# neuraloperator/neuraloperator

Hardware: AMD Instinct MI355X
Metric: FNO SpectralConv fwd+bwd samples/sec (higher is better)
Workload: dtype f32; 1 GPU; fno2d_256_m64_c64_b32; B_per_gpu=32, global_batch=32, channels=64, parallelism=single, launch=eager, real_tensor_io=f32, weights=dense complex64, random init

## Files before the change

include/sc_engine.h:

```cpp
#ifndef SC_ENGINE_H
#define SC_ENGINE_H

#include <stddef.h>
#include <stdint.h>

#ifdef __cplusplus
extern "C" {
#endif

#define SC_MAX_DIMS 4

enum { SC_NORM_FORWARD = 0, SC_NORM_BACKWARD = 1, SC_NORM_ORTHO = 2 };

enum {
  SC_FWD_SCALED = 0,
  SC_FWD_ADJ_C2R = 1,
  SC_INV_PADDED = 0,
  SC_INV_ADJ_R2C = 1
};

typedef struct sc_plan sc_plan;

typedef struct {
  int32_t ndim;
// ... 20 lines not shown
};

int sc_plan_create(sc_plan** out, const sc_plan_desc* desc);
void sc_plan_destroy(sc_plan* plan);
size_t sc_plan_workspace_bytes(const sc_plan* plan, int64_t n_images);
int sc_plan_is_fast(const sc_plan* plan);

int sc_transform_forward(const sc_plan* plan, int mode, const float* x, float* xhat,
                         int64_t n_images, void* workspace, void* stream);

int sc_transform_inverse(const sc_plan* plan, int mode, const float* yhat, const float* bias,
                         int64_t channels, float* y, int64_t n_images, void* workspace,
                         void* stream);

enum {
  SC_GEMM_FORCE_VALU = 1,
  SC_GEMM_STREAM_C = 2,
  SC_GEMM_PAIRED = 4,
  SC_GEMM_WIDE = 8,
  SC_GEMM_NO_STREAM = 16,
  SC_GEMM_NO_SB = 64,
  SC_GEMM_SB_WM4 = 128,
  SC_GEMM_SB_ALT_ORDER = 1 << 25,
  SC_GEMM_NO_FMX = 1 << 24,
  SC_GEMM_F16 = 32
};
#define SC_GEMM_GRID(n) (((n) & 0xffff) << 8)

typedef struct {
  int64_t P, Q, R, n_modes;
  int64_t a_sp, a_sr, a_sm;
  int64_t b_sr, b_sq, b_sm;
  int64_t c_sp, c_sq, c_sm;
  int32_t conj_a, conj_b;
  int32_t accumulate;
  int32_t flags;
  const int32_t* b_idx;
  const int32_t* c_idx;
  int64_t a_sg, b_sg, c_sg;
} sc_modegemm_desc;

int sc_modegemm(const sc_modegemm_desc* d, const float* A, const float* B, float* C,
                void* stream);
int sc_modegemm_pair(const sc_modegemm_desc* d0, const float* A0, const float* B0, float* C0,
                     const sc_modegemm_desc* d1, const float* A1, const float* B1, float* C1, void* stream);
int sc_modegemm_pair_fused(const sc_modegemm_desc* d0, const sc_modegemm_desc* d1);
int sc_modegemm_pair_path(const sc_modegemm_desc* d0, const sc_modegemm_desc* d1);
int sc_modegemm_msum(const sc_modegemm_desc* d, const float* A, const float* B, float* C,
                     void* stream);
size_t sc_modegemm_msum_workspace_bytes(const sc_modegemm_desc* d);
int sc_modegemm_msum_ws(const sc_modegemm_desc* d, const float* A, const float* B, float* C, void* workspace,
                        size_t workspace_bytes, void* stream);
int sc_modegemm_msum_path(const sc_modegemm_desc* d);
int sc_modegemm_uses_matrix_cores(const sc_modegemm_desc* d);
int sc_modegemm_path(const sc_modegemm_desc* d);

int sc_round_f16(const float* in, float* out, int64_t n, void* stream);

int sc_wire_pack_c32(const float* spec, void* wire, int64_t n, int64_t c, int64_t k1, int64_t rest, int64_t P,
                     int64_t rows, int64_t w0, void* stream);

int sc_wire_unpack_c32(const void* wire, float* spec, int64_t n, int64_t c, int64_t k1, int64_t rest, int64_t P,
                       int64_t rows, int64_t w0, void* stream);

int sc_bicubic_rows_forward(const float* x, float* y, int64_t images, int64_t rows_in, int64_t w_in, int64_t src_row0,
                            int64_t h_in, int64_t h_out, int64_t w_out, int64_t out_row0, int64_t rows_out, void* stream);
int sc_bicubic_rows_backward(const float* gy, float* gx, int64_t images, int64_t rows_in, int64_t w_in, int64_t src_row0,
                             int64_t h_in, int64_t h_out, int64_t w_out, int64_t out_row0, int64_t rows_out, void* stream);
// ... 187 lines not shown
```

neuraloperator_amd/_lib.py:

```python
import atexit
import ctypes
import os
import sys
from ctypes import (POINTER, Structure, byref, c_char_p, c_int, c_int32, c_int64, c_size_t,
                    c_void_p)

SC_MAX_DIMS = 4
SC_NORM = {"forward": 0, "backward": 1, "ortho": 2}
SC_FWD_SCALED, SC_FWD_ADJ_C2R = 0, 1
SC_INV_PADDED, SC_INV_ADJ_R2C = 0, 1
SC_PLAN_FORCE_GENERIC = 1
SC_PLAN_FFT_GEN2 = 2
SC_PLAN_NO_MDFT = 4
SC_PLAN_COMPLEX = 8
SC_PLAN_IO_BF16 = 16
SC_PLAN_NO_F2P_SMALL = 32
SC_PLAN_F2P_SMALL_ALWAYS = 64
SC_PLAN_NO_SPAN = 128
SC_PLAN_NO_MX_FFT = 256
SC_PLAN_MX_FFT_3TERM = 512
SC_FREQ_DROPPED = -(1 << 63)
SC_GEMM_FORCE_VALU = 1
SC_GEMM_STREAM_C = 2
SC_GEMM_PAIRED = 4
SC_GEMM_WIDE = 8
SC_GEMM_NO_STREAM = 16
SC_GEMM_F16 = 32
SC_GEMM_NO_SB = 64
SC_GEMM_SB_WM4 = 128
SC_GEMM_NO_FMX = 1 << 24
SC_GEMM_SB_ALT_ORDER = 1 << 25


def SC_GEMM_GRID(n):
    return (int(n) & 0xffff) << 8

_HERE = os.path.dirname(os.path.abspath(__file__))
DEFAULT_LIB = os.path.join(_HERE, "libsc_engine.so")


class PlanDesc(Structure):
    _fields_ = [("ndim", c_int32), ("fft_norm", c_int32),
                ("spatial", c_int64 * SC_MAX_DIMS), ("kept", c_int64 * SC_MAX_DIMS),
                ("flags", c_int32), ("real_col", c_int32),
                ("freq", POINTER(c_int64) * SC_MAX_DIMS)]


class AdamwDesc(Structure):
    _fields_ = [("lr", ctypes.c_double), ("beta1", ctypes.c_double), ("beta2", ctypes.c_double),
                ("eps", ctypes.c_double), ("weight_decay", ctypes.c_double), ("step", c_int64),
                ("correct_bias", c_int32), ("reserved", c_int32)]


class SpectrumShards(Structure):
# ... 84 lines not shown
        ptr, self._as_parameter_ = self._as_parameter_, None
        try:
            if ptr is not None and self._lib is not None and not _SHUTDOWN and not _finalizing():
                self._lib.sc_plan_destroy(ptr)
        except Exception:
            pass

    def __del__(self):
        self.destroy()


class ScEngineLib:

    SYMBOLS = ["sc_plan_create", "sc_plan_destroy", "sc_plan_workspace_bytes", "sc_plan_is_fast",
               "sc_transform_forward", "sc_transform_inverse", "sc_modegemm",
               "sc_modegemm_msum", "sc_modegemm_msum_ws", "sc_modegemm_msum_workspace_bytes", "sc_modegemm_msum_path", "sc_modegemm_uses_matrix_cores", "sc_modegemm_path", "sc_bias_grad", "sc_adamw_step",
               "sc_layer_workspace_bytes", "sc_layer_forward", "sc_layer_backward",
               "sc_last_error", "sc_version", "sc_plan_kernel_name", "sc_transform_inverse_ex",
               "sc_layer_forward_ex", "sc_round_f16", "sc_pointwise_mlp_forward", "sc_pointwise_block_forward",
               "sc_pointwise_mlp_backward", "sc_pointwise_mlp_workspace_bytes", "sc_pointwise_linear_forward",
               "sc_pointwise_linear_backward", "sc_pointwise_linear_workspace_bytes", "sc_layer_backward_ex",
               "sc_pointwise_mlp_backward_ex", "sc_tucker_modes_supported", "sc_tucker_modes_forward",
               "sc_tucker_modes_backward", "sc_tucker_modes_workspace_bytes", "sc_modegemm_pair",
               "sc_modegemm_pair_fused", "sc_modegemm_pair_path", "sc_plan_workspace_bytes_sharded", "sc_transform_forward_sharded",
               "sc_transform_inverse_sharded", "sc_bias_grad_sharded", "sc_tucker_chain_forward",
               "sc_tucker_chain_backward", "sc_tucker_chain_workspace_bytes", "sc_tucker_chain_fused_supported",
               "sc_tucker_chain_t3m_bytes", "sc_tucker_chain_forward_fused", "sc_tucker_chain_backward_fused",
               "sc_tucker_chain_backward_fused_workspace_bytes", "sc_peer_window_alloc", "sc_peer_window_open",
               "sc_peer_window_close", "sc_peer_window_free", "sc_peer_all_to_all", "sc_peer_window_control", "sc_pointwise_linear_forward_ex",
               "sc_pointwise_linear_workspace_bytes_ex", "sc_pointwise_linear_backward_ex", "sc_pointwise_block_backward",
               "sc_pointwise_block_backward_supported", "sc_bicubic_rows_forward", "sc_bicubic_rows_backward",
               "sc_wire_pack_c32", "sc_wire_unpack_c32", "sc_legendre_analysis", "sc_legendre_synthesis", "sc_spectral_op"]

    def __init__(self, path=DEFAULT_LIB):
        if not os.path.isfile(path):
            raise EngineError(
                f"{path} not found: the HIP engine is not built. Run "
                "`python -c 'import __graft_entry__ as g; g.build()'` (needs hipcc). "
                "There is no fallback path.")
        self.path = path
        self.lib = ctypes.CDLL(path)
        L = self.lib
        for s in self.SYMBOLS:
            if not hasattr(L, s):
                raise EngineError(f"{path} does not export {s}")
        L.sc_plan_create.argtypes = [POINTER(c_void_p), POINTER(PlanDesc)]
        L.sc_plan_create.restype = c_int
        L.sc_plan_destroy.argtypes = [c_void_p]
        L.sc_plan_destroy.restype = None
        L.sc_plan_workspace_bytes.argtypes = [c_void_p, c_int64]
        L.sc_plan_workspace_bytes.restype = c_size_t
        L.sc_plan_is_fast.argtypes = [c_void_p]
        L.sc_plan_is_fast.restype = c_int
        L.sc_transform_forward.argtypes = [c_void_p, c_int, c_void_p, c_void_p, c_int64,
                                           c_void_p, c_void_p]
        L.sc_transform_forward.restype = c_int
        L.sc_transform_inverse.argtypes = [c_void_p, c_int, c_void_p, c_void_p, c_int64,
                                           c_void_p, c_int64, c_void_p, c_void_p]
        L.sc_transform_inverse.restype = c_int
        L.sc_modegemm.argtypes = [POINTER(ModeGemmDesc), c_void_p, c_void_p, c_void_p, c_void_p]
        L.sc_modegemm.restype = c_int
        L.sc_modegemm_pair.argtypes = [POINTER(ModeGemmDesc), c_void_p, c_void_p, c_void_p,
                                       POINTER(ModeGemmDesc), c_void_p, c_void_p, c_void_p, c_void_p]
        L.sc_modegemm_pair.restype = c_int
        L.sc_modegemm_pair_fused.argtypes = [POINTER(ModeGemmDesc), POINTER(ModeGemmDesc)]
        L.sc_modegemm_pair_fused.restype = c_int
        L.sc_modegemm_pair_path.argtypes = [POINTER(ModeGemmDesc), POINTER(ModeGemmDesc)]
        L.sc_modegemm_pair_path.restype = c_int
        L.sc_modegemm_msum.argtypes = [POINTER(ModeGemmDesc), c_void_p, c_void_p, c_void_p, c_void_p]
        L.sc_modegemm_msum.restype = c_int
        L.sc_modegemm_msum_workspace_bytes.argtypes = [POINTER(ModeGemmDesc)]
        L.sc_modegemm_msum_workspace_bytes.restype = c_size_t
        L.sc_modegemm_msum_ws.argtypes = [POINTER(ModeGemmDesc), c_void_p, c_void_p, c_void_p, c_void_p, c_size_t, c_void_p]
        L.sc_modegemm_msum_ws.restype = c_int
        L.sc_modegemm_msum_path.argtypes = [POINTER(ModeGemmDesc)]
        L.sc_modegemm_msum_path.restype = c_int
        L.sc_modegemm_uses_matrix_cores.argtypes = [POINTER(ModeGemmDesc)]
        L.sc_modegemm_uses_matrix_cores.restype = c_int
        L.sc_modegemm_path.argtypes = [POINTER(ModeGemmDesc)]
        L.sc_modegemm_path.restype = c_int
        L.sc_bias_grad.argtypes = [c_void_p, c_void_p, c_int64, c_int64, c_void_p, c_void_p]
        L.sc_bias_grad.restype = c_int
        L.sc_plan_workspace_bytes_sharded.argtypes = [c_void_p, c_int64]
        L.sc_plan_workspace_bytes_sharded.restype = c_size_t
        L.sc_transform_forward_sharded.argtypes = [c_void_p, c_int, c_void_p, c_void_p, c_int64,
                                                   POINTER(SpectrumShards), c_void_p, c_void_p]
        L.sc_transform_forward_sharded.restype = c_int
# ... 174 lines not shown

    def modegemm(self, a_ptr, b_ptr, c_ptr, stream=0, **kw):
        self._check(self.lib.sc_modegemm(byref(self._gemm_desc(kw)), a_ptr, b_ptr, c_ptr, stream))

    _DESC_CACHE = {}

    @staticmethod
    def _gemm_desc(kw):
        key = tuple(kw.items())
        d = ScEngineLib._DESC_CACHE.get(key)
        if d is None:
            if len(ScEngineLib._DESC_CACHE) > 4096:
                ScEngineLib._DESC_CACHE.clear()
            d = ModeGemmDesc()
            for k, v in kw.items():
                setattr(d, k, v)
            ScEngineLib._DESC_CACHE[key] = d
        return d

    def modegemm_pair(self, kw0, a0, b0, c0, kw1, a1, b1, c1, stream=0):
        d0, d1 = self._gemm_desc(kw0), self._gemm_desc(kw1)
        self._check(self.lib.sc_modegemm_pair(byref(d0), a0, b0, c0, byref(d1), a1, b1, c1, stream))

    def modegemm_pair_fused(self, kw0, kw1):
        d0, d1 = self._gemm_desc(kw0), self._gemm_desc(kw1)
        return bool(self.lib.sc_modegemm_pair_fused(byref(d0), byref(d1)))

    def modegemm_pair_path(self, kw0, kw1):
        d0, d1 = self._gemm_desc(kw0), self._gemm_desc(kw1)
        return int(self.lib.sc_modegemm_pair_path(byref(d0), byref(d1)))

    def pointwise_mlp_forward(self, batch, c_in, c_hid, c_out, spatial, act, x, w1, b1, w2, b2, skip, gate, out, stream=0):
        d = PmlpDesc(batch, c_in, c_hid, c_out, spatial, act, 0)
        self._check(self.lib.sc_pointwise_mlp_forward(byref(d), x, w1, b1, w2, b2, skip, gate, out, stream))

    def pointwise_mlp_workspace_bytes(self, batch, c_in, c_hid, c_out, spatial, act):
        d = PmlpDesc(batch, c_in, c_hid, c_out, spatial, act, 0)
        return int(self.lib.sc_pointwise_mlp_workspace_bytes(byref(d)))

    def pointwise_block_forward(self, batch, c, c_hid, spatial, act, conv, x, ws, bs, w1, b1, w2, b2, gate, y, pre, out,
                                stream=0):
        d = PmlpDesc(batch, c, c_hid, c, spatial, act, 0)
        self._check(self.lib.sc_pointwise_block_forward(byref(d), conv, x, ws, bs, w1, b1, w2, b2, gate, y, pre, out, stream))

    def pointwise_mlp_backward(self, batch, c_in, c_hid, c_out, spatial, act, x, w1, b1, w2, b2, skip, gate, gout,
                               gx, gw1, gb1, gw2, gb2, gskip, ggate, ws, stream=0, x_pre=0):
# ... 224 lines not shown
```

neuraloperator_amd/csrc/sc_engine.cpp:

```cpp
#include <atomic>
#include "../../include/sc_engine.h"

#include <cmath>
#include <cstdio>
#include <cstdlib>
#include <cstring>
#include <map>
#include <mutex>
#include <string>
#include <vector>

#include "sc_device.h"
#ifdef SC_DIAG
#define SC_DIAG_ENV(name) std::getenv(name)
#else
#define SC_DIAG_ENV(name) ((const char*)nullptr)
#endif
#include "sc_kernels_generic.h"
#include "sc_kernels_fft.h"
#include "sc_kernels_fft3.h"
#include "sc_kernels_fft3mx.h"
#include "sc_kernels_mfma.h"
#include "sc_kernels_gemm8.h"
#include "sc_kernels_mdft.h"
// ... 1900 lines not shown
#define SC_G8_RESIDENT(wide) ((wide) ? 512 : SC_G8_NARROW_RESIDENT)
static bool gemm8_eligible(const sc_modegemm_desc* d, const void* A, const void* B, const void* C) {
  if (d->flags & (SC_GEMM_FORCE_VALU | SC_GEMM_NO_STREAM | SC_GEMM_F16)) return false;
  if (d->accumulate || d->b_idx || d->c_idx) return false;
  if (d->a_sm != 1 || d->b_sm != 1 || d->c_sm != 1) return false;
  if (d->n_modes % 8 != 0 || d->n_modes >= ((int64_t)1 << 31)) return false;
  if ((d->a_sg || d->b_sg || d->c_sg) && d->n_modes % 16 != 0) return false;
  if ((d->a_sg | d->b_sg | d->c_sg) & 1) return false;
  if ((d->a_sp | d->a_sr | d->b_sr | d->b_sq | d->c_sp | d->c_sq) & 1) return false;
  if (((uintptr_t)A | (uintptr_t)B | (uintptr_t)C) & 15) return false;
  const int64_t cols = 32;
  const int64_t Pp = (d->P + 31) / 32 * 32, Qp = (d->Q + cols - 1) / cols * cols;
  static const int64_t fill4 = [] { const char* e = SC_DIAG_ENV("SC_G8_FILL4"); return e ? (int64_t)std::atoi(e) : (int64_t)2; }();
  bool rows_ok = 4 * d->P >= fill4 * Pp;
  if (d->P >= 8 && d->P <= 32 && d->b_sq > d->b_sr) rows_ok = true;
  if (!rows_ok || 4 * d->Q < fill4 * Qp) return false;
  if (d->R < 4) return false;
  if (Pp / 32 * (Qp / cols) * (d->n_modes / 8) >= ((int64_t)1 << 30)) return false;
  return true;
}

template <int GS, int QT, int SUB, int D, bool IL, bool CA, bool CB>
static void launch_gemm8(const Gemm8Args& g, const cf32* A, const cf32* B, cf32* C, sc_stream_t st) {
  SC_LAUNCH((k_modegemm_dma<GS, QT, SUB, D, IL, CA, CB>), dim3((unsigned)g.G), dim3((Gemm8Cfg<GS, QT, SUB>::THREADS)),
            0, st, g, A, B, C);
}

template <int GS, int QT, int SUB, int D, bool IL>
static void dispatch_gemm8(const Gemm8Args& g, int ca, int cb, const cf32* A, const cf32* B, cf32* C, sc_stream_t st) {
  if (!ca && !cb) launch_gemm8<GS, QT, SUB, D, IL, false, false>(g, A, B, C, st);
  else if (ca && !cb) launch_gemm8<GS, QT, SUB, D, IL, true, false>(g, A, B, C, st);
  else if (!ca && cb) launch_gemm8<GS, QT, SUB, D, IL, false, true>(g, A, B, C, st);
  else launch_gemm8<GS, QT, SUB, D, IL, true, true>(g, A, B, C, st);
}

static bool gemm8_args(const sc_modegemm_desc* d, Gemm8Args& g, int64_t resident_narrow, int64_t resident_wide,
                       int force_shape ) {
  const int64_t cols = 32;
  const int64_t tiles = ((d->P + 31) / 32) * ((d->Q + cols - 1) / cols);
  bool wide;
  if (force_shape >= 0) wide = force_shape == 1;
  else {
#if defined(SC_G8_FORCE_NARROW)
    wide = false;
#elif defined(SC_G8_FORCE_WIDE)
    wide = d->n_modes % 16 == 0;
#else
// ... 7 lines not shown
  g.n_pb = (int)((d->P + 31) / 32);
  g.n_qb = (int)((d->Q + cols - 1) / cols);
  g.a_sp = d->a_sp; g.a_sr = d->a_sr;
  g.b_sr = d->b_sr; g.b_sq = d->b_sq;
  g.c_sp = d->c_sp; g.c_sq = d->c_sq;
  g.a_sg = d->a_sg ? d->a_sg : 16;
  g.b_sg = d->b_sg ? d->b_sg : 16;
  g.c_sg = d->c_sg ? d->c_sg : 16;
  g.stream_c = (d->flags & SC_GEMM_STREAM_C) ? 1 : 0;
  const int64_t nblk = (int64_t)g.n_pb * g.n_qb;
  int64_t bpw = 1;
  if (g.n_mg <= resident && g.n_mg * nblk > resident) {
    bpw = nblk;
    for (int64_t b = 1; b <= nblk; ++b)
      if (g.n_mg * ((nblk + b - 1) / b) <= resident) {
        bpw = b;
        break;
      }
  }
  const int64_t cap = (d->flags >> 8) & 0xffff;
  if (cap > 0 && cap <= nblk) bpw = cap;
  g.bpw = (int)bpw;
  g.G = (int)(g.n_mg * ((nblk + bpw - 1) / bpw));
  return wide;
}

static int run_gemm8(const sc_modegemm_desc* d, const cf32* A, const cf32* B, cf32* C, sc_stream_t st) {
  Gemm8Args g;
  const bool wide = gemm8_args(d, g, SC_G8_RESIDENT(false), SC_G8_RESIDENT(true), -1);
  if (wide) dispatch_gemm8<SC_G8_WIDE>(g, d->conj_a, d->conj_b, A, B, C, st);
  else dispatch_gemm8<SC_G8_NARROW>(g, d->conj_a, d->conj_b, A, B, C, st);
  return sc_check_launch("k_modegemm_dma");
}

#ifndef SC_G8_PAIR_BPW
#define SC_G8_PAIR_BPW 0
#endif
static void gemm8_pair_args(const sc_modegemm_desc* d0, const sc_modegemm_desc* d1, Gemm8Args& g0, Gemm8Args& g1) {
  gemm8_args(d0, g0, SC_G8_RESIDENT(false), SC_G8_RESIDENT(true), 0);
  gemm8_args(d1, g1, SC_G8_RESIDENT(false), SC_G8_RESIDENT(true), 0);
  for (Gemm8Args* g : {&g0, &g1}) {
    g->bpw = 1;
    g->G = (int)((int64_t)g->n_mg * g->n_pb * g->n_qb);
  }
#if SC_G8_PAIR_BPW >= 1
  g0.bpw = g0.n_pb * g0.n_qb; g0.G = g0.n_mg;
#endif
#if SC_G8_PAIR_BPW == 1
  g1.bpw = g1.n_pb * g1.n_qb; g1.G = g1.n_mg;
#endif
}

static int run_gemm8_bwd(const sc_modegemm_desc* d0, const cf32* A0, const cf32* B0, cf32* C0,
                         const sc_modegemm_desc* d1, const cf32* A1, const cf32* B1, cf32* C1,
                         const Gemm8Bias& bias, sc_stream_t st) {
#ifdef SC_G8_NO_PAIR
  return -1;
#endif
  if (!gemm8_eligible(d0, A0, B0, C0) || !gemm8_eligible(d1, A1, B1, C1)) return -1;
  if (!(d0->conj_a && !d0->conj_b && !d1->conj_a && d1->conj_b)) return -1;
  if (d0->n_modes != d1->n_modes) return -1;
  Gemm8Args g0, g1;
#ifdef SC_G8_PAIR_NARROW_ONLY
  if (gemm8_args(d0, g0, SC_G8_RESIDENT(false), SC_G8_RESIDENT(true), -1) ||
      gemm8_args(d1, g1, SC_G8_RESIDENT(false), SC_G8_RESIDENT(true), -1)) return -1;
#endif
  gemm8_pair_args(d0, d1, g0, g1);
  if ((g0.G & 7) || (g1.G & 7)) return -1;
  typedef Gemm8Cfg<4, 2, 2> K;
  const int64_t nb = bias.ghat ? (bias.channels + K::NW - 1) / K::NW : 0;
  if ((int64_t)g0.G + g1.G + nb >= ((int64_t)1 << 30)) return -1;
  SC_LAUNCH((k_modegemm_dma_bwd<SC_G8_NARROW>), dim3((unsigned)(g0.G + g1.G + nb)), dim3(K::THREADS), 0, st,
            g0, A0, B0, C0, g1, A1, B1, C1, bias);
  return sc_check_launch("k_modegemm_dma_bwd");
}

extern "C" int sc_modegemm(const sc_modegemm_desc* d, const float* A, const float* B, float* C,
                           void* stream) {
  SC_CHECK_ARG(d && A && B && C, "null argument");
  SC_CHECK_ARG(d->P >= 0 && d->Q >= 0 && d->R >= 0 && d->n_modes >= 0, "negative extent");
  if (d->P == 0 || d->Q == 0 || d->n_modes == 0) return 0;
  SC_CHECK_ARG(d->R > 0, "R must be > 0");
  ModeGemmArgs g;
  g.P = d->P; g.Q = d->Q; g.R = d->R; g.M = d->n_modes;
  g.a_sp = d->a_sp; g.a_sr = d->a_sr; g.a_sm = d->a_sm;
  g.b_sr = d->b_sr; g.b_sq = d->b_sq; g.b_sm = d->b_sm;
  g.c_sp = d->c_sp; g.c_sq = d->c_sq; g.c_sm = d->c_sm;
  g.b_idx = d->b_idx; g.c_idx = d->c_idx;
  g.accumulate = d->accumulate;
  SC_CHECK_ARG(((g.M + 63) / 64) * ((g.P + 15) / 16) * ((g.Q + 3) / 4) < ((int64_t)1 << 30),
               "problem too large for one launch grid");
  sc_stream_t st = (sc_stream_t)stream;
  const cf32* a = (const cf32*)A;
  const cf32* b = (const cf32*)B;
  cf32* c = (cf32*)C;
  if (d->flags & SC_GEMM_F16) {
    SC_CHECK_ARG(!d->accumulate && !(d->a_sg || d->b_sg || d->c_sg), "SC_GEMM_F16: plain C = A B launches only");
    g.n_mt = (int)((g.M + SC_WAVE - 1) / SC_WAVE);
    g.n_pg = (int)((g.P + 15) / 16);
    g.n_qt = (int)((g.Q + 3) / 4);
    g.per_xcd = 0;
    const dim3 grid((unsigned)((int64_t)g.n_mt * g.n_pg * g.n_qt));
    if (d->conj_a && d->conj_b) SC_LAUNCH((k_modegemm_f16<true, true>), grid, dim3(SC_BLOCK), 0, st, g, a, b, c);
    else if (d->conj_a) SC_LAUNCH((k_modegemm_f16<true, false>), grid, dim3(SC_BLOCK), 0, st, g, a, b, c);
    else if (d->conj_b) SC_LAUNCH((k_modegemm_f16<false, true>), grid, dim3(SC_BLOCK), 0, st, g, a, b, c);
    else SC_LAUNCH((k_modegemm_f16<false, false>), grid, dim3(SC_BLOCK), 0, st, g, a, b, c);
    return sc_check_launch("k_modegemm_f16");
  }
  if (fmx_bfac_eligible(d)) return run_fmx_bfac(d, a, b, c, st);
  if (bfac_gemm_eligible(d)) {
    const int rc = run_bfac_gemm(d, a, b, c, st);
    if (rc >= 0) return rc;
  }
  if (sb_gemm_eligible(d, A, B, C)) {
    const int rc = run_sb_gemm(d, a, b, c, st);
    if (rc >= 0) return rc;
  }
  if (gemm8_eligible(d, A, B, C)) return run_gemm8(d, a, b, c, st);
  SC_CHECK_ARG(!(d->a_sg || d->b_sg || d->c_sg),
               "tiled operands (a_sg / b_sg / c_sg) need the streamed matrix-core kernel: n_modes % 16 == 0, unit mode "
               "strides, no index tables, 16-byte aligned rows, near-full 32 x 32 tiles");
  if (!(d->flags & SC_GEMM_FORCE_VALU) && mfma_gemm_eligible(d))
    return run_mfma_gemm(d, a, b, c, st);
  if (g.Q > 4) return dispatch_modegemm_conj<4, 8>(g, d->conj_a, d->conj_b, a, b, c, st);
  return dispatch_modegemm_conj<4, 4>(g, d->conj_a, d->conj_b, a, b, c, st);
}

extern "C" int sc_modegemm_pair(const sc_modegemm_desc* d0, const float* A0, const float* B0, float* C0,
                                const sc_modegemm_desc* d1, const float* A1, const float* B1, float* C1,
                                void* stream) {
  SC_CHECK_ARG(d0 && d1 && A0 && B0 && C0 && A1 && B1 && C1, "null argument");
  if (d0->P > 0 && d0->Q > 0 && d0->R > 0 && d0->n_modes > 0 && d1->P > 0 && d1->Q > 0 && d1->R > 0) {
    Gemm8Bias nobias;
    std::memset(&nobias, 0, sizeof(nobias));
    int rc = run_sb_bwd(d0, (const cf32*)A0, (const cf32*)B0, (cf32*)C0, d1, (const cf32*)A1, (const cf32*)B1, (cf32*)C1,
                        (sc_stream_t)stream);
    if (rc >= 0) return rc;
    rc = run_gemm8_bwd(d0, (const cf32*)A0, (const cf32*)B0, (cf32*)C0, d1, (const cf32*)A1,
                       (const cf32*)B1, (cf32*)C1, nobias, (sc_stream_t)stream);
    if (rc >= 0) return rc;
  }
  const int rc = sc_modegemm(d0, A0, B0, C0, stream);
  return rc ? rc : sc_modegemm(d1, A1, B1, C1, stream);
}

extern "C" int sc_modegemm_pair_path(const sc_modegemm_desc* d0, const sc_modegemm_desc* d1) {
  if (!d0 || !d1) return 0;
  static const float* const al = reinterpret_cast<const float*>(uintptr_t(256));
  if (sb_bwd_eligible(d0, al, al, al, d1, al, al, al)) return 2;
  return sc_modegemm_pair_fused(d0, d1) ? 1 : 0;
}

extern "C" int sc_modegemm_pair_fused(const sc_modegemm_desc* d0, const sc_modegemm_desc* d1) {
  if (!d0 || !d1) return 0;
#ifdef SC_G8_NO_PAIR
  return 0;
#else
  static const float* const al = reinterpret_cast<const float*>(uintptr_t(256));
  if (!gemm8_eligible(d0, al, al, al) || !gemm8_eligible(d1, al, al, al)) return 0;
  if (!(d0->conj_a && !d0->conj_b && !d1->conj_a && d1->conj_b) || d0->n_modes != d1->n_modes) return 0;
  Gemm8Args g0, g1;
  gemm8_pair_args(d0, d1, g0, g1);
  return !((g0.G & 7) || (g1.G & 7));
#endif
}

// ... 1551 lines not shown
```

neuraloperator_amd/csrc/sc_kernels_gemm8.h:

```cpp
#pragma once
#include "sc_device.h"
#include "sc_kernels_mfma.h"

struct Gemm8Args {
  int P, Q, R;
  int n_mg, n_pb, n_qb, bpw;
  int G;
  int64_t a_sp, a_sr, b_sr, b_sq, c_sp, c_sq;
  int64_t a_sg, b_sg, c_sg;
  int stream_c;
};

template <int GS, int QT, int SUB = 1>
struct Gemm8Cfg {
  static constexpr int NW = GS;
  static constexpr int THREADS = 64 * NW;
  static constexpr int MODES = 2 * GS;
  static constexpr int COLS = 16 * QT;
  static constexpr int SP = 64 / GS;
  static constexpr int SH = (GS == 4) ? 2 : 1;
  static constexpr int A_G = 2 * 32 * GS;
  static constexpr int B_G = 2 * COLS * GS;
  static constexpr int SUB_G = A_G + B_G;
  static constexpr int STAGE_G = SUB * SUB_G;
  static constexpr int NPA = A_G / 64, NPB = B_G / 64;
  static constexpr int PPW = SUB * (NPA + NPB) / NW;
  static constexpr int RP = 2048 / (16 * GS);
  static constexpr int EPW = 32 / GS;
  static constexpr int occupancy(const int D) {
    const int wgs = 163840 / (D * STAGE_G * 16);
// ... 7 lines not shown

#ifdef SC_G8_NO_3M
#define SC_G8_USE_3M(GS, QT, IL) false
#else
#define SC_G8_USE_3M(GS, QT, IL) ((GS) == 4 && (QT) == 2 && !(IL))
#endif

#ifndef SC_EMU
SC_DEVICE void sc_store16(cf32* dst, const sc_f4 v, const int stream) {
  if (stream) __builtin_nontemporal_store(v, reinterpret_cast<sc_f4*>(dst));
  else *reinterpret_cast<sc_f4*>(dst) = v;
}
#else
inline void sc_store16(cf32* dst, const sc_f4 v, const int) { std::memcpy(dst, &v, 16); }
#endif

template <int NEWER, int PPW>
SC_DEVICE void g8_wait_stage(const int newer_issued) {
  static_assert(NEWER >= 0 && NEWER * PPW <= 63, "vmcnt range");
  if (newer_issued >= NEWER) sc_wait_vmcnt<NEWER * PPW>();
  else sc_wait_vmcnt<0>();
}

template <int GS, int QT, int SUB, int D, bool IL, bool CA, bool CB>
SC_DEVICE void g8_workgroup(const Gemm8Args& g, const cf32* __restrict__ A, const cf32* __restrict__ B,
                            cf32* __restrict__ C, int gid, sc_f4* lds) {
  typedef Gemm8Cfg<GS, QT, SUB> K;
  static_assert(D * K::STAGE_G >= 2048, "the epilogue patch (32 KiB) lives in the ring");

  const int tid = SC_TID, lane = tid & 63;
  const int w = SC_UNIFORM(tid >> 6);
  const int nblk = g.n_pb * g.n_qb;
  const int chunks = (nblk + g.bpw - 1) / g.bpw;
  if ((g.G & 7) == 0) gid = (gid & 7) * (g.G >> 3) + (gid >> 3);
  const int mg = gid / chunks, ch = gid - mg * chunks;
  constexpr int GPG = 16 / K::MODES;
  const int64_t mlo = (int64_t)(mg % GPG) * K::MODES;
  const int64_t mA = (int64_t)(mg / GPG) * g.a_sg + mlo, mB = (int64_t)(mg / GPG) * g.b_sg + mlo,
                mC = (int64_t)(mg / GPG) * g.c_sg + mlo;

  const int ls = lane / GS, ltq = lane % GS;
  constexpr int APR = 32 / K::SP, BPR = K::COLS / K::SP;
  constexpr int NBW = K::NPB / K::NW;
  const int ra_k = w / APR, ra_g = w % APR;
  const int rowA = ra_g * K::SP + ls;
  const int lgrA = ltq ^ ((rowA >> K::SH) & (GS - 1));
  const int kk = lane >> 5, li = lane & 31, d = lane & 1, qq = li >> 1;
  const int a_g = (kk * 32 + li) * GS + (w ^ ((li >> K::SH) & (GS - 1)));
  const int b_g = K::A_G + (kk * K::COLS + qq) * GS + (w ^ ((qq >> K::SH) & (GS - 1)));
  constexpr bool M3 = SC_G8_USE_3M(GS, QT, IL);
  constexpr int NB = M3 ? 1 : QT;
  constexpr bool FLIP = CB && !M3;
  constexpr bool CAe = FLIP ? !CA : CA, CBe = FLIP ? false : CB;
  const int b_g3 = K::A_G + (kk * K::COLS + li) * GS + (w ^ ((li >> K::SH) & (GS - 1)));
  const uint32_t m_re = (CBe && d) ? 0x80000000u : 0u;
  const uint32_t m_im = (!CBe && !d) ? 0x80000000u : 0u;
  const uint32_t dsel = d ? 0xffffffffu : 0u;
  const int NS = (g.R + 2 * SUB - 1) / (2 * SUB);

  const int b_end = (ch + 1) * g.bpw < nblk ? (ch + 1) * g.bpw : nblk;
#pragma unroll 1
  for (int bi = ch * g.bpw; bi < b_end; ++bi) {
    const int pb = bi / g.n_qb, qb = bi - pb * g.n_qb;
    const int p0 = pb * 32, q0 = qb * K::COLS;
    int prow = p0 + rowA;
    prow = prow < g.P ? prow : g.P - 1;
    const cf32* srcA = A + (int64_t)prow * g.a_sp + mA + 2 * lgrA;
    const cf32* srcB[NBW];
    int rb_k[NBW];
#pragma unroll
    for (int j = 0; j < NBW; ++j) {
      const int kb = w + K::NW * j;
      rb_k[j] = kb / BPR;
      const int colB = (kb % BPR) * K::SP + ls;
      int qcol = q0 + colB;
      qcol = qcol < g.Q ? qcol : g.Q - 1;
      srcB[j] = B + (int64_t)qcol * g.b_sq + mB + 2 * (ltq ^ ((colB >> K::SH) & (GS - 1)));
    }
    const int64_t stepA = 2 * g.a_sr, stepB = 2 * g.b_sr;
    const cf32* pA = srcA + (int64_t)ra_k * g.a_sr;
    const cf32* pB[NBW];
#pragma unroll
    for (int j = 0; j < NBW; ++j) pB[j] = srcB[j] + (int64_t)rb_k[j] * g.b_sr;
    int r_next = 0;
    auto issue_piece = [&](const int buf, const int pc) {
      sc_f4* sb = lds + buf * K::STAGE_G;
      const int sub = pc / (1 + NBW), e = pc % (1 + NBW);
      if (e == 0) {
        const int64_t backA = (r_next + ra_k < g.R) ? 0 : (int64_t)(r_next + ra_k - (g.R - 1)) * g.a_sr;
        SC_GLDS16(pA - backA, sb + sub * K::SUB_G + w * 64);
        pA += stepA;
      }
#pragma unroll
      for (int j = 0; j < NBW; ++j)
        if (e == 1 + j) {
          const int64_t backB = (r_next + rb_k[j] < g.R) ? 0 : (int64_t)(r_next + rb_k[j] - (g.R - 1)) * g.b_sr;
          SC_GLDS16(pB[j] - backB, sb + sub * K::SUB_G + K::A_G + (w + K::NW * j) * 64);
          pB[j] += stepB;
        }
      if (e == NBW) r_next += 2;
    };
    auto issue = [&](const int buf) {
#pragma unroll
      for (int pc = 0; pc < K::PPW; ++pc) issue_piece(buf, pc);
    };
    struct Ops {
      sc_f4 a;
      sc_f4 b[NB];
    };
    auto fetch = [&](const int buf, Ops (&o)[SUB]) {
#pragma unroll
      for (int sub = 0; sub < SUB; ++sub) {
        const sc_f4* sb = lds + buf * K::STAGE_G + sub * K::SUB_G;
        o[sub].a = sb[a_g];
        if constexpr (M3) o[sub].b[0] = sb[b_g3];
        else {
#pragma unroll
          for (int u = 0; u < QT; ++u) o[sub].b[u] = sb[b_g + u * 16 * GS];
// ... 37 lines not shown
        asm volatile("" ::"v"(q.br[0][u]), "v"(q.br[1][u]), "v"(q.bm[0][u]), "v"(q.bm[1][u]), "v"(q.ar[0]), "v"(q.ai[1]));
      return;
#endif
      SC_SCHED_BARRIER();
#pragma unroll
      for (int u = 0; u < QT; ++u) {
        sc_mfma_32x32x2(acc[0][u], q.ar[0], q.br[0][u]);
        sc_mfma_32x32x2(acc[1][u], q.ar[1], q.br[1][u]);
      }
#pragma unroll
      for (int u = 0; u < QT; ++u) {
        sc_mfma_32x32x2(acc[0][u], q.ai[0], q.bm[0][u]);
        sc_mfma_32x32x2(acc[1][u], q.ai[1], q.bm[1][u]);
      }
      SC_SCHED_BARRIER();
    };

    if constexpr (!IL) {
    sc_wait_vmcnt<0>();
    const int npro = NS < D - 1 ? NS : D - 1;
    for (int st = 0; st < npro; ++st) issue(st);
#pragma unroll 1
    for (int st = 0; st < NS; ++st) {
      g8_wait_stage<D - 2, K::PPW>(NS - 1 - st);
      SC_WAIT_LGKM0();
      SC_BARRIER_RAW();
      if (st + D - 1 < NS) issue((st + D - 1) % D);
      Ops o[SUB];
      fetch(st % D, o);
#pragma unroll
      for (int sub = 0; sub < SUB; ++sub) {
        if constexpr (M3) {
          const int r0 = 2 * (st * SUB + sub);
          const float keep = (r0 + kk < g.R) ? 1.f : 0.f;
          const sc_f4 a = o[sub].a, b = o[sub].b[0];
          const float ar0 = a.x * keep, ai0 = (CA ? -a.y : a.y) * keep, ar1 = a.z * keep, ai1 = (CA ? -a.w : a.w) * keep;
          const float bi0 = CB ? -b.y : b.y, bi1 = CB ? -b.w : b.w;
#ifdef SC_G8_ABL_NOMFMA
          asm volatile("" ::"v"(ar0 + ai0), "v"(ar1 + ai1), "v"(b.x + bi0), "v"(b.z + bi1));
#else
          SC_SCHED_BARRIER();
          sc_mfma_32x32x2(acc[0][0], ar0, b.x);
          sc_mfma_32x32x2(acc[1][0], ar1, b.z);
          sc_mfma_32x32x2(acc[0][1], ai0, bi0);
          sc_mfma_32x32x2(acc[1][1], ai1, bi1);
          sc_mfma_32x32x2(acc[0][2], ar0 + ai0, b.x + bi0);
          sc_mfma_32x32x2(acc[1][2], ar1 + ai1, b.z + bi1);
// ... 42 lines not shown
        } else if (m < K::PPW + NF) {
          const int f = m - K::PPW, fs = f / (1 + QT), fe = f % (1 + QT);
          if (more) {
            if (fe == 0) on[fs].a = sbn[fs * K::SUB_G + a_g];
            else on[fs].b[fe - 1] = sbn[fs * K::SUB_G + b_g + (fe - 1) * 16 * GS];
          }
        } else if (m < K::PPW + NF + SUB) {
          const int ps = m - K::PPW - NF;
          if (more) prep(on[ps], 2 * ((st + 1) * SUB + ps), qn[ps]);
        }
        SC_SCHED_BARRIER();
      }
    };
#pragma unroll 1
    for (int st = 0; st < NS; st += 2) {
      stage(st, q0, q1);
      if (st + 1 < NS) stage(st + 1, q1, q0);
    }
    }

    float* patch = reinterpret_cast<float*>(lds);
    SC_WAIT_LGKM0();
    SC_BARRIER_RAW();
    const bool full = p0 + 32 <= g.P && q0 + K::COLS <= g.Q;
    if constexpr (M3) {
      static_assert(K::RP == 32 && K::COLS == 32, "3-product epilogue: 32 x 32 tiles, 32 KiB patches");
      const int pslot3 = (li * GS + (w ^ ((li >> K::SH) & (GS - 1)))) * 4;
#pragma unroll
      for (int h = 0; h < 2; ++h) {
        if (h) SC_BARRIER_RAW();
#pragma unroll
        for (int j = 0; j < 2; ++j)
#pragma unroll
          for (int v = 0; v < 16; ++v) {
            const int row = (v & 3) + 8 * (v >> 2);
            if (row / 16 == h) {
              const float p1 = acc[j][0][v], p2 = acc[j][1][v], p3 = acc[j][2][v];
              float* dst = patch + pslot3 + ((row % 16) + 4 * kk) * (128 * GS) + 2 * j;
              dst[0] = p1 - p2;
              dst[1] = (p3 - p1) - p2;
            }
          }
        SC_WAIT_LGKM0();
        SC_BARRIER_RAW();
        sc_f4 val[K::EPW];
#pragma unroll
        for (int e = 0; e < K::EPW; ++e) val[e] = lds[(w * K::EPW + e) * 64 + lane];
#pragma unroll
        for (int e = 0; e < K::EPW; ++e) {
          const int sbase = (w * K::EPW + e) * K::SP;
          const int prow_ = p0 + h * 16 + (sbase >> 5);
          const int col = (sbase & 31) + sc_opaque(ls);
          const int qc = q0 + col;
          const int gr = ltq ^ ((col >> K::SH) & (GS - 1));
#ifdef SC_G8_ABL_NOSTORE
          asm volatile("" ::"v"(val[e]));
          if (g.P < 0)
#endif
          if (full || (prow_ < g.P && qc < g.Q))
            sc_store16(C + (int64_t)prow_ * g.c_sp + (int64_t)qc * g.c_sq + mC + 2 * gr, val[e], g.stream_c);
        }
      }
    } else {
      const int pslot = ((w ^ ((qq >> K::SH) & (GS - 1))) * 4 + d) + qq * 4 * GS;
      bool first = true;
#pragma unroll
      for (int u = 0; u < QT; ++u) {
#pragma unroll
        for (int h = 0; h < 32 / K::RP; ++h) {
          if (!first) SC_BARRIER_RAW();
          first = false;
#pragma unroll
// ... 21 lines not shown
            const int prow_ = p0 + h * K::RP + (sbase >> 4);
            const int col = (sbase & 15) + sc_opaque(ls);
            const int qc = q0 + u * 16 + col;
            const int gr = ltq ^ ((col >> K::SH) & (GS - 1));
#ifdef SC_G8_ABL_NOSTORE
            asm volatile("" ::"v"(val[e]));
            if (g.P < 0)
#endif
            if (full || (prow_ < g.P && qc < g.Q))
              sc_store16(C + (int64_t)prow_ * g.c_sp + (int64_t)qc * g.c_sq + mC + 2 * gr, val[e], g.stream_c);
          }
        }
      }
    }
    SC_WAIT_LGKM0();
    SC_BARRIER_RAW();
  }
}

template <int GS, int QT, int SUB, int D, bool IL, bool CA, bool CB>
SC_GLOBAL void SC_LAUNCH_BOUNDS_OCC((Gemm8Cfg<GS, QT, SUB>::THREADS), (Gemm8Cfg<GS, QT, SUB>::occupancy(D)))
k_modegemm_dma(Gemm8Args g, const cf32* __restrict__ A, const cf32* __restrict__ B, cf32* __restrict__ C) {
  SC_SHARED __attribute__((aligned(16))) sc_f4 lds[D * Gemm8Cfg<GS, QT, SUB>::STAGE_G];
  g8_workgroup<GS, QT, SUB, D, IL, CA, CB>(g, A, B, C, SC_BID_X, lds);
}

struct Gemm8Bias {
  const cf32* ghat;
  float* gbias;
  int64_t batch, channels, modes_per_image, dc;
};

template <int GS, int QT, int SUB, int D, bool IL>
SC_GLOBAL void SC_LAUNCH_BOUNDS_OCC((Gemm8Cfg<GS, QT, SUB>::THREADS), (Gemm8Cfg<GS, QT, SUB>::occupancy(D)))
k_modegemm_dma_bwd(Gemm8Args g0, const cf32* __restrict__ A0, const cf32* __restrict__ B0, cf32* __restrict__ C0,
                   Gemm8Args g1, const cf32* __restrict__ A1, const cf32* __restrict__ B1, cf32* __restrict__ C1,
                   Gemm8Bias bias) {
  typedef Gemm8Cfg<GS, QT, SUB> K;
  SC_SHARED __attribute__((aligned(16))) sc_f4 lds[D * K::STAGE_G];
  const int b = SC_BID_X;
  const int n0 = g0.G >> 3, n1 = g1.G >> 3;
  const int oct = b >> 3, l8 = b & 7;
  if (oct < n0 + n1) {
    const int len0 = ((g0.R + 2 * SUB - 1) / (2 * SUB)) * g0.bpw, len1 = ((g1.R + 2 * SUB - 1) / (2 * SUB)) * g1.bpw;
    const int first = len1 > len0 ? 1 : 0, nf = first ? n1 : n0;
    const int job = oct < nf ? first : 1 - first;
    const int k = (oct < nf ? oct : oct - nf) * 8 + l8;
    if (job) g8_workgroup<GS, QT, SUB, D, IL, false, true>(g1, A1, B1, C1, k, lds);
    else g8_workgroup<GS, QT, SUB, D, IL, true, false>(g0, A0, B0, C0, k, lds);
  } else {
    const int tid = SC_TID, lane = tid & 63, w = tid >> 6;
    const int64_t c = (int64_t)(b - 8 * (n0 + n1)) * K::NW + w;
    if (c < bias.channels)
      sc_bias_grad_wave(bias.ghat, bias.gbias, bias.batch, bias.channels, bias.modes_per_image, bias.dc, c, lane,
                        reinterpret_cast<float*>(lds) + 64 * w);
  }
}
```

Before: 63980 samples/s.

## Split tail-wave GEMM tiles into half-width workgroups to balance the last wave

Adds a tail scheduler to the matrix-core mode GEMM. When the tile count is not a multiple of the CU count, the last k*rem tiles are each split into two half-width (16-column) workgroups, so the final partial wave is spread across more CUs. The grid size becomes F + 2*(G-F), and both the single and the paired backward kernels remap block ids through a slot function. Half-width tiles load only half of B and store half of the epilogue, which adds extra A traffic and per-tile overhead in exchange for less tail imbalance.

```diff
diff --git a/include/sc_engine.h b/include/sc_engine.h
--- a/include/sc_engine.h
+++ b/include/sc_engine.h
@@ -66,6 +66,7 @@
   SC_GEMM_NO_SB = 64,
   SC_GEMM_SB_WM4 = 128,
   SC_GEMM_SB_ALT_ORDER = 1 << 25,
+  SC_GEMM_UNIFORM_GRID = 1 << 26,
   SC_GEMM_NO_FMX = 1 << 24,
   SC_GEMM_F16 = 32
 };
@@ -86,8 +87,14 @@
 
 int sc_modegemm(const sc_modegemm_desc* d, const float* A, const float* B, float* C,
                 void* stream);
+int sc_modegemm_sched(const sc_modegemm_desc* d, const float* A, const float* B, float* C, int64_t full_tiles,
+                      void* stream);
+int sc_modegemm_full_tiles(const sc_modegemm_desc* d, int64_t* tiles);
 int sc_modegemm_pair(const sc_modegemm_desc* d0, const float* A0, const float* B0, float* C0,
                      const sc_modegemm_desc* d1, const float* A1, const float* B1, float* C1, void* stream);
+int sc_modegemm_pair_sched(const sc_modegemm_desc* d0, const float* A0, const float* B0, float* C0,
+                           const sc_modegemm_desc* d1, const float* A1, const float* B1, float* C1,
+                           int64_t full_tiles, void* stream);
 int sc_modegemm_pair_fused(const sc_modegemm_desc* d0, const sc_modegemm_desc* d1);
 int sc_modegemm_pair_path(const sc_modegemm_desc* d0, const sc_modegemm_desc* d1);
 int sc_modegemm_msum(const sc_modegemm_desc* d, const float* A, const float* B, float* C,
diff --git a/neuraloperator_amd/_lib.py b/neuraloperator_amd/_lib.py
--- a/neuraloperator_amd/_lib.py
+++ b/neuraloperator_amd/_lib.py
@@ -30,6 +30,7 @@
 SC_GEMM_SB_WM4 = 128
 SC_GEMM_NO_FMX = 1 << 24
 SC_GEMM_SB_ALT_ORDER = 1 << 25
+SC_GEMM_UNIFORM_GRID = 1 << 26
 
 
 def SC_GEMM_GRID(n):
@@ -160,7 +161,8 @@
                "sc_pointwise_linear_backward", "sc_pointwise_linear_workspace_bytes", "sc_layer_backward_ex",
                "sc_pointwise_mlp_backward_ex", "sc_tucker_modes_supported", "sc_tucker_modes_forward",
                "sc_tucker_modes_backward", "sc_tucker_modes_workspace_bytes", "sc_modegemm_pair",
-               "sc_modegemm_pair_fused", "sc_modegemm_pair_path", "sc_plan_workspace_bytes_sharded", "sc_transform_forward_sharded",
+               "sc_modegemm_pair_fused", "sc_modegemm_pair_path", "sc_modegemm_sched", "sc_modegemm_pair_sched",
+               "sc_modegemm_full_tiles", "sc_plan_workspace_bytes_sharded", "sc_transform_forward_sharded",
                "sc_transform_inverse_sharded", "sc_bias_grad_sharded", "sc_tucker_chain_forward",
                "sc_tucker_chain_backward", "sc_tucker_chain_workspace_bytes", "sc_tucker_chain_fused_supported",
                "sc_tucker_chain_t3m_bytes", "sc_tucker_chain_forward_fused", "sc_tucker_chain_backward_fused",
@@ -201,6 +203,13 @@
         L.sc_modegemm_pair.argtypes = [POINTER(ModeGemmDesc), c_void_p, c_void_p, c_void_p,
                                        POINTER(ModeGemmDesc), c_void_p, c_void_p, c_void_p, c_void_p]
         L.sc_modegemm_pair.restype = c_int
+        L.sc_modegemm_sched.argtypes = [POINTER(ModeGemmDesc), c_void_p, c_void_p, c_void_p, c_int64, c_void_p]
+        L.sc_modegemm_sched.restype = c_int
+        L.sc_modegemm_pair_sched.argtypes = [POINTER(ModeGemmDesc), c_void_p, c_void_p, c_void_p,
+                                             POINTER(ModeGemmDesc), c_void_p, c_void_p, c_void_p, c_int64, c_void_p]
+        L.sc_modegemm_pair_sched.restype = c_int
+        L.sc_modegemm_full_tiles.argtypes = [POINTER(ModeGemmDesc), POINTER(c_int64)]
+        L.sc_modegemm_full_tiles.restype = c_int
         L.sc_modegemm_pair_fused.argtypes = [POINTER(ModeGemmDesc), POINTER(ModeGemmDesc)]
         L.sc_modegemm_pair_fused.restype = c_int
         L.sc_modegemm_pair_path.argtypes = [POINTER(ModeGemmDesc), POINTER(ModeGemmDesc)]
@@ -421,6 +430,18 @@
         d0, d1 = self._gemm_desc(kw0), self._gemm_desc(kw1)
         self._check(self.lib.sc_modegemm_pair(byref(d0), a0, b0, c0, byref(d1), a1, b1, c1, stream))
 
+    def modegemm_sched(self, a_ptr, b_ptr, c_ptr, full_tiles, stream=0, **kw):
+        self._check(self.lib.sc_modegemm_sched(byref(self._gemm_desc(kw)), a_ptr, b_ptr, c_ptr, full_tiles, stream))
+
+    def modegemm_pair_sched(self, kw0, a0, b0, c0, kw1, a1, b1, c1, full_tiles, stream=0):
+        d0, d1 = self._gemm_desc(kw0), self._gemm_desc(kw1)
+        self._check(self.lib.sc_modegemm_pair_sched(byref(d0), a0, b0, c0, byref(d1), a1, b1, c1, full_tiles, stream))
+
+    def modegemm_full_tiles(self, **kw):
+        t = c_int64(0)
+        f = int(self.lib.sc_modegemm_full_tiles(byref(self._gemm_desc(kw)), byref(t)))
+        return f, int(t.value)
+
     def modegemm_pair_fused(self, kw0, kw1):
         d0, d1 = self._gemm_desc(kw0), self._gemm_desc(kw1)
         return bool(self.lib.sc_modegemm_pair_fused(byref(d0), byref(d1)))
diff --git a/neuraloperator_amd/csrc/sc_engine.cpp b/neuraloperator_amd/csrc/sc_engine.cpp
--- a/neuraloperator_amd/csrc/sc_engine.cpp
+++ b/neuraloperator_amd/csrc/sc_engine.cpp
@@ -1946,7 +1946,7 @@
 
 template <int GS, int QT, int SUB, int D, bool IL, bool CA, bool CB>
 static void launch_gemm8(const Gemm8Args& g, const cf32* A, const cf32* B, cf32* C, sc_stream_t st) {
-  SC_LAUNCH((k_modegemm_dma<GS, QT, SUB, D, IL, CA, CB>), dim3((unsigned)g.G), dim3((Gemm8Cfg<GS, QT, SUB>::THREADS)),
+  SC_LAUNCH((k_modegemm_dma<GS, QT, SUB, D, IL, CA, CB>), dim3((unsigned)g8_grid(g)), dim3((Gemm8Cfg<GS, QT, SUB>::THREADS)),
             0, st, g, A, B, C);
 }
 
@@ -2000,12 +2000,40 @@
   if (cap > 0 && cap <= nblk) bpw = cap;
   g.bpw = (int)bpw;
   g.G = (int)(g.n_mg * ((nblk + bpw - 1) / bpw));
+  g.F = g.G;
   return wide;
 }
 
-static int run_gemm8(const sc_modegemm_desc* d, const cf32* A, const cf32* B, cf32* C, sc_stream_t st) {
+#ifndef SC_G8_TAIL_K
+#define SC_G8_TAIL_K 0
+#endif
+static void gemm8_full_tiles(Gemm8Args& g, bool wide, int32_t flags, int64_t resident, int64_t force_full) {
+  g.F = g.G;
+#ifdef SC_G8_NO_3M
+  return;
+#endif
+  if (wide || g.bpw != 1 || (flags & SC_GEMM_UNIFORM_GRID)) return;
+  if (force_full >= 0) {
+    g.F = (int)(force_full < g.G ? force_full : g.G);
+    return;
+  }
+  static const int64_t k_env = [] { const char* e = SC_DIAG_ENV("SC_G8_TAIL_K"); return e ? (int64_t)std::atoi(e) : (int64_t)-1; }();
+  int64_t k = k_env >= 0 ? k_env : SC_G8_TAIL_K;
+  const int64_t cus = sc_cu_count(), rem = g.G % cus;
+  if (g.G <= cus || g.G > resident || rem == 0) return;
+  if (2 * k * rem > cus) k = 1;
+  if (2 * k * rem > cus) return;
+  int64_t full = g.G - k * rem;
+  if ((g.G & 7) == 0) full &= ~(int64_t)7;
+  if (2 * (g.G - full) > cus) return;
+  g.F = (int)full;
+}
+
+static int run_gemm8(const sc_modegemm_desc* d, const cf32* A, const cf32* B, cf32* C, sc_stream_t st,
+                     int64_t force_full = -1) {
   Gemm8Args g;
   const bool wide = gemm8_args(d, g, SC_G8_RESIDENT(false), SC_G8_RESIDENT(true), -1);
+  gemm8_full_tiles(g, wide, d->flags, SC_G8_RESIDENT(wide), force_full);
   if (wide) dispatch_gemm8<SC_G8_WIDE>(g, d->conj_a, d->conj_b, A, B, C, st);
   else dispatch_gemm8<SC_G8_NARROW>(g, d->conj_a, d->conj_b, A, B, C, st);
   return sc_check_launch("k_modegemm_dma");
@@ -2031,7 +2059,7 @@
 
 static int run_gemm8_bwd(const sc_modegemm_desc* d0, const cf32* A0, const cf32* B0, cf32* C0,
                          const sc_modegemm_desc* d1, const cf32* A1, const cf32* B1, cf32* C1,
-                         const Gemm8Bias& bias, sc_stream_t st) {
+                         const Gemm8Bias& bias, sc_stream_t st, int64_t force_full = -1) {
 #ifdef SC_G8_NO_PAIR
   return -1;
 #endif
@@ -2045,16 +2073,34 @@
 #endif
   gemm8_pair_args(d0, d1, g0, g1);
   if ((g0.G & 7) || (g1.G & 7)) return -1;
+  gemm8_full_tiles(g1, false, d0->flags | d1->flags, SC_G8_RESIDENT(false), force_full);
   typedef Gemm8Cfg<4, 2, 2> K;
   const int64_t nb = bias.ghat ? (bias.channels + K::NW - 1) / K::NW : 0;
-  if ((int64_t)g0.G + g1.G + nb >= ((int64_t)1 << 30)) return -1;
-  SC_LAUNCH((k_modegemm_dma_bwd<SC_G8_NARROW>), dim3((unsigned)(g0.G + g1.G + nb)), dim3(K::THREADS), 0, st,
+  const int64_t grid = g8_grid(g0) + g8_grid(g1) + nb;
+  if (grid >= ((int64_t)1 << 30)) return -1;
+  SC_LAUNCH((k_modegemm_dma_bwd<SC_G8_NARROW>), dim3((unsigned)grid), dim3(K::THREADS), 0, st,
             g0, A0, B0, C0, g1, A1, B1, C1, bias);
   return sc_check_launch("k_modegemm_dma_bwd");
 }
 
 extern "C" int sc_modegemm(const sc_modegemm_desc* d, const float* A, const float* B, float* C,
                            void* stream) {
+  return sc_modegemm_sched(d, A, B, C, -1, stream);
+}
+
+extern "C" int sc_modegemm_full_tiles(const sc_modegemm_desc* d, int64_t* tiles) {
+  if (tiles) *tiles = 0;
+  if (!d || sc_modegemm_path(d) != 2) return -1;
+  Gemm8Args g;
+  const bool wide = gemm8_args(d, g, SC_G8_RESIDENT(false), SC_G8_RESIDENT(true), -1);
+  if (wide || g.bpw != 1) return -1;
+  gemm8_full_tiles(g, wide, d->flags, SC_G8_RESIDENT(wide), -1);
+  if (tiles) *tiles = g.G;
+  return g.F;
+}
+
+extern "C" int sc_modegemm_sched(const sc_modegemm_desc* d, const float* A, const float* B, float* C,
+                                 int64_t full_tiles, void* stream) {
   SC_CHECK_ARG(d && A && B && C, "null argument");
   SC_CHECK_ARG(d->P >= 0 && d->Q >= 0 && d->R >= 0 && d->n_modes >= 0, "negative extent");
   if (d->P == 0 || d->Q == 0 || d->n_modes == 0) return 0;
@@ -2094,7 +2140,7 @@
     const int rc = run_sb_gemm(d, a, b, c, st);
     if (rc >= 0) return rc;
   }
-  if (gemm8_eligible(d, A, B, C)) return run_gemm8(d, a, b, c, st);
+  if (gemm8_eligible(d, A, B, C)) return run_gemm8(d, a, b, c, st, full_tiles);
   SC_CHECK_ARG(!(d->a_sg || d->b_sg || d->c_sg),
                "tiled operands (a_sg / b_sg / c_sg) need the streamed matrix-core kernel: n_modes % 16 == 0, unit mode "
                "strides, no index tables, 16-byte aligned rows, near-full 32 x 32 tiles");
@@ -2107,6 +2153,12 @@
 extern "C" int sc_modegemm_pair(const sc_modegemm_desc* d0, const float* A0, const float* B0, float* C0,
                                 const sc_modegemm_desc* d1, const float* A1, const float* B1, float* C1,
                                 void* stream) {
+  return sc_modegemm_pair_sched(d0, A0, B0, C0, d1, A1, B1, C1, -1, stream);
+}
+
+extern "C" int sc_modegemm_pair_sched(const sc_modegemm_desc* d0, const float* A0, const float* B0, float* C0,
+                                      const sc_modegemm_desc* d1, const float* A1, const float* B1, float* C1,
+                                      int64_t full_tiles, void* stream) {
   SC_CHECK_ARG(d0 && d1 && A0 && B0 && C0 && A1 && B1 && C1, "null argument");
   if (d0->P > 0 && d0->Q > 0 && d0->R > 0 && d0->n_modes > 0 && d1->P > 0 && d1->Q > 0 && d1->R > 0) {
     Gemm8Bias nobias;
@@ -2115,11 +2167,11 @@
                         (sc_stream_t)stream);
     if (rc >= 0) return rc;
     rc = run_gemm8_bwd(d0, (const cf32*)A0, (const cf32*)B0, (cf32*)C0, d1, (const cf32*)A1,
-                       (const cf32*)B1, (cf32*)C1, nobias, (sc_stream_t)stream);
+                       (const cf32*)B1, (cf32*)C1, nobias, (sc_stream_t)stream, full_tiles);
     if (rc >= 0) return rc;
   }
   const int rc = sc_modegemm(d0, A0, B0, C0, stream);
-  return rc ? rc : sc_modegemm(d1, A1, B1, C1, stream);
+  return rc ? rc : sc_modegemm_sched(d1, A1, B1, C1, full_tiles, stream);
 }
 
 extern "C" int sc_modegemm_pair_path(const sc_modegemm_desc* d0, const sc_modegemm_desc* d1) {
diff --git a/neuraloperator_amd/csrc/sc_kernels_gemm8.h b/neuraloperator_amd/csrc/sc_kernels_gemm8.h
--- a/neuraloperator_amd/csrc/sc_kernels_gemm8.h
+++ b/neuraloperator_amd/csrc/sc_kernels_gemm8.h
@@ -6,6 +6,7 @@
   int P, Q, R;
   int n_mg, n_pb, n_qb, bpw;
   int G;
+  int F;
   int64_t a_sp, a_sr, b_sr, b_sq, c_sp, c_sq;
   int64_t a_sg, b_sg, c_sg;
   int stream_c;
@@ -59,11 +60,35 @@
   else sc_wait_vmcnt<0>();
 }
 
-template <int GS, int QT, int SUB, int D, bool IL, bool CA, bool CB>
+struct Gemm8Slot {
+  int pos, half;
+};
+SC_DEVICE Gemm8Slot g8_slot(const Gemm8Args& g, const int b) {
+  Gemm8Slot s;
+  if (b < g.F) {
+    s.pos = b;
+    s.half = -1;
+  } else {
+    const int h = b - g.F;
+    if (((g.F | g.G) & 7) == 0) {
+      s.pos = g.F + (h >> 4) * 8 + (h & 7);
+      s.half = (h >> 3) & 1;
+    } else {
+      s.pos = g.F + (h >> 1);
+      s.half = h & 1;
+    }
+  }
+  return s;
+}
+SC_HD int64_t g8_grid(const Gemm8Args& g) { return (int64_t)g.F + 2 * ((int64_t)g.G - g.F); }
+
+template <int GS, int QT, int SUB, int D, bool IL, bool CA, bool CB, bool HF = false>
 SC_DEVICE void g8_workgroup(const Gemm8Args& g, const cf32* __restrict__ A, const cf32* __restrict__ B,
-                            cf32* __restrict__ C, int gid, sc_f4* lds) {
+                            cf32* __restrict__ C, int gid, sc_f4* lds, const int hq = 0) {
   typedef Gemm8Cfg<GS, QT, SUB> K;
   static_assert(D * K::STAGE_G >= 2048, "the epilogue patch (32 KiB) lives in the ring");
+  static_assert(!HF || (SC_G8_USE_3M(GS, QT, IL) && K::SP == 16 && K::NPB / K::NW == 1),
+                "half-width tiles: the three-product shape, one 16-column B piece per wave");
 
   const int tid = SC_TID, lane = tid & 63;
   const int w = SC_UNIFORM(tid >> 6);
@@ -89,7 +114,9 @@
   constexpr int NB = M3 ? 1 : QT;
   constexpr bool FLIP = CB && !M3;
   constexpr bool CAe = FLIP ? !CA : CA, CBe = FLIP ? false : CB;
-  const int b_g3 = K::A_G + (kk * K::COLS + li) * GS + (w ^ ((li >> K::SH) & (GS - 1)));
+  const int lc = HF ? (li & 15) : li;
+  const int b_g3 = K::A_G + (kk * K::COLS + lc) * GS + (w ^ ((lc >> K::SH) & (GS - 1)));
+  const bool ldB = !HF || !(w & 1);
   const uint32_t m_re = (CBe && d) ? 0x80000000u : 0u;
   const uint32_t m_im = (!CBe && !d) ? 0x80000000u : 0u;
   const uint32_t dsel = d ? 0xffffffffu : 0u;
@@ -99,7 +126,8 @@
 #pragma unroll 1
   for (int bi = ch * g.bpw; bi < b_end; ++bi) {
     const int pb = bi / g.n_qb, qb = bi - pb * g.n_qb;
-    const int p0 = pb * 32, q0 = qb * K::COLS;
+    const int p0 = pb * 32, q0 = qb * K::COLS + (HF ? 16 * hq : 0);
+    if (HF && q0 >= g.Q) return;
     int prow = p0 + rowA;
     prow = prow < g.P ? prow : g.P - 1;
     const cf32* srcA = A + (int64_t)prow * g.a_sp + mA + 2 * lgrA;
@@ -130,7 +158,7 @@
       }
 #pragma unroll
       for (int j = 0; j < NBW; ++j)
-        if (e == 1 + j) {
+        if (e == 1 + j && ldB) {
           const int64_t backB = (r_next + rb_k[j] < g.R) ? 0 : (int64_t)(r_next + rb_k[j] - (g.R - 1)) * g.b_sr;
           SC_GLDS16(pB[j] - backB, sb + sub * K::SUB_G + K::A_G + (w + K::NW * j) * 64);
           pB[j] += stepB;
@@ -214,7 +242,8 @@
     for (int st = 0; st < npro; ++st) issue(st);
 #pragma unroll 1
     for (int st = 0; st < NS; ++st) {
-      g8_wait_stage<D - 2, K::PPW>(NS - 1 - st);
+      if (ldB) g8_wait_stage<D - 2, K::PPW>(NS - 1 - st);
+      else g8_wait_stage<D - 2, SUB>(NS - 1 - st);
       SC_WAIT_LGKM0();
       SC_BARRIER_RAW();
       if (st + D - 1 < NS) issue((st + D - 1) % D);
@@ -303,7 +332,7 @@
     float* patch = reinterpret_cast<float*>(lds);
     SC_WAIT_LGKM0();
     SC_BARRIER_RAW();
-    const bool full = p0 + 32 <= g.P && q0 + K::COLS <= g.Q;
+    const bool full = p0 + 32 <= g.P && q0 + (HF ? 16 : K::COLS) <= g.Q;
     if constexpr (M3) {
       static_assert(K::RP == 32 && K::COLS == 32, "3-product epilogue: 32 x 32 tiles, 32 KiB patches");
       const int pslot3 = (li * GS + (w ^ ((li >> K::SH) & (GS - 1)))) * 4;
@@ -315,7 +344,7 @@
 #pragma unroll
           for (int v = 0; v < 16; ++v) {
             const int row = (v & 3) + 8 * (v >> 2);
-            if (row / 16 == h) {
+            if (row / 16 == h && (!HF || li < 16)) {
               const float p1 = acc[j][0][v], p2 = acc[j][1][v], p3 = acc[j][2][v];
               float* dst = patch + pslot3 + ((row % 16) + 4 * kk) * (128 * GS) + 2 * j;
               dst[0] = p1 - p2;
@@ -326,9 +355,11 @@
         SC_BARRIER_RAW();
         sc_f4 val[K::EPW];
 #pragma unroll
-        for (int e = 0; e < K::EPW; ++e) val[e] = lds[(w * K::EPW + e) * 64 + lane];
+        for (int e = 0; e < K::EPW; ++e)
+          if (!HF || !(e & 1)) val[e] = lds[(w * K::EPW + e) * 64 + lane];
 #pragma unroll
         for (int e = 0; e < K::EPW; ++e) {
+          if (HF && (e & 1)) continue;
           const int sbase = (w * K::EPW + e) * K::SP;
           const int prow_ = p0 + h * 16 + (sbase >> 5);
           const int col = (sbase & 31) + sc_opaque(ls);
@@ -396,6 +427,13 @@
 SC_GLOBAL void SC_LAUNCH_BOUNDS_OCC((Gemm8Cfg<GS, QT, SUB>::THREADS), (Gemm8Cfg<GS, QT, SUB>::occupancy(D)))
 k_modegemm_dma(Gemm8Args g, const cf32* __restrict__ A, const cf32* __restrict__ B, cf32* __restrict__ C) {
   SC_SHARED __attribute__((aligned(16))) sc_f4 lds[D * Gemm8Cfg<GS, QT, SUB>::STAGE_G];
+  if constexpr (SC_G8_USE_3M(GS, QT, IL)) {
+    const Gemm8Slot s = g8_slot(g, SC_BID_X);
+    if (s.half >= 0) {
+      g8_workgroup<GS, QT, SUB, D, IL, CA, CB, true>(g, A, B, C, s.pos, lds, s.half);
+      return;
+    }
+  }
   g8_workgroup<GS, QT, SUB, D, IL, CA, CB>(g, A, B, C, SC_BID_X, lds);
 }
 
@@ -412,19 +450,34 @@
                    Gemm8Bias bias) {
   typedef Gemm8Cfg<GS, QT, SUB> K;
   SC_SHARED __attribute__((aligned(16))) sc_f4 lds[D * K::STAGE_G];
-  const int b = SC_BID_X;
-  const int n0 = g0.G >> 3, n1 = g1.G >> 3;
-  const int oct = b >> 3, l8 = b & 7;
-  if (oct < n0 + n1) {
-    const int len0 = ((g0.R + 2 * SUB - 1) / (2 * SUB)) * g0.bpw, len1 = ((g1.R + 2 * SUB - 1) / (2 * SUB)) * g1.bpw;
-    const int first = len1 > len0 ? 1 : 0, nf = first ? n1 : n0;
-    const int job = oct < nf ? first : 1 - first;
-    const int k = (oct < nf ? oct : oct - nf) * 8 + l8;
-    if (job) g8_workgroup<GS, QT, SUB, D, IL, false, true>(g1, A1, B1, C1, k, lds);
-    else g8_workgroup<GS, QT, SUB, D, IL, true, false>(g0, A0, B0, C0, k, lds);
+  int b = SC_BID_X;
+  const int len0 = ((g0.R + 2 * SUB - 1) / (2 * SUB)) * g0.bpw, len1 = ((g1.R + 2 * SUB - 1) / (2 * SUB)) * g1.bpw;
+  const int first = len1 > len0 ? 1 : 0;
+  const int nf = (int)g8_grid(first ? g1 : g0), ns = (int)g8_grid(first ? g0 : g1);
+#ifdef SC_G8_PAIR_HALVES_LAST
+  if (b < nf + ns) {
+    const int ff = first ? g1.F : g0.F;
+    if (b >= ff) b = b < ff + ns ? b - ff + nf : b - ns;
+  }
+#endif
+  if (b < nf + ns) {
+    const int job = b < nf ? first : 1 - first;
+    Gemm8Slot s;
+    s.pos = b < nf ? b : b - nf;
+    s.half = -1;
+    if constexpr (SC_G8_USE_3M(GS, QT, IL)) {
+      s = g8_slot(job ? g1 : g0, s.pos);
+      if (s.half >= 0) {
+        if (job) g8_workgroup<GS, QT, SUB, D, IL, false, true, true>(g1, A1, B1, C1, s.pos, lds, s.half);
+        else g8_workgroup<GS, QT, SUB, D, IL, true, false, true>(g0, A0, B0, C0, s.pos, lds, s.half);
+        return;
+      }
+    }
+    if (job) g8_workgroup<GS, QT, SUB, D, IL, false, true>(g1, A1, B1, C1, s.pos, lds);
+    else g8_workgroup<GS, QT, SUB, D, IL, true, false>(g0, A0, B0, C0, s.pos, lds);
   } else {
     const int tid = SC_TID, lane = tid & 63, w = tid >> 6;
-    const int64_t c = (int64_t)(b - 8 * (n0 + n1)) * K::NW + w;
+    const int64_t c = (int64_t)(b - (nf + ns)) * K::NW + w;
     if (c < bias.channels)
       sc_bias_grad_wave(bias.ghat, bias.gbias, bias.batch, bias.channels, bias.modes_per_image, bias.dc, c, lane,
                         reinterpret_cast<float*>(lds) + 64 * w);
```

Result: slower. 62540 samples/s (-2.2%).
